# X1X1010/XequiNet

Hardware: AMD Instinct MI355X
Metric: edges/sec + achieved HBM GB/s, energy+force inference, QM9-shape batch (higher is better)
Workload: dtype f32

## Files before the change

### include/xeq.h

```cpp
#ifndef XEQ_H
#define XEQ_H
#include <stdint.h>

#ifdef __cplusplus
extern "C" {
#endif

enum { XEQ_F32 = 0, XEQ_F64 = 1 };
enum { XEQ_RBF_BESSEL = 0, XEQ_RBF_GAUSSIAN = 1, XEQ_RBF_EXPBERN = 2, XEQ_RBF_EXPNORM = 3 };
enum { XEQ_CUTOFF_COSINE = 0, XEQ_CUTOFF_POLYNOMIAL = 1 };
enum {
  XEQ_OK = 0,
  XEQ_ERR_INVALID_ARGUMENT = 1,
  XEQ_ERR_LAUNCH = 2,
  XEQ_ERR_UNSUPPORTED = 3
};

int xeq_version(void);
const char* xeq_last_error(void);
int64_t xeq_launch_count(void);
int64_t xeq_launch_names(int64_t first, char* buf, int64_t cap);


int xeq_csr_rowptr(const int64_t* keys, int64_t n_keys, int64_t n_rows, int32_t* rowptr, void* stream);
// ... 119 lines not shown
int xeq_wgrad_chunks(int64_t n, int m, int k);
int xeq_wgrad(const void* a, int64_t lda, const void* b, int64_t ldb, int64_t n, int m, int k, int with_bias, int n_chunks, void* parts,
              void* stream);

int xeq_load_padded_batch(int dtype, const void* pos, const int32_t* z, const int64_t* ptr, const int64_t* batch, int64_t n,
                          int64_t g, int64_t n_cap, int64_t g_cap, double pad0, double spacing, void* pos_out, int32_t* z_out,
                          int64_t* ptr_out, int64_t* batch_out, void* stream);
int xeq_load_padded_batch_z64(int dtype, const void* pos, const int64_t* z, const int64_t* ptr, const int64_t* batch, int64_t n, int64_t g,
                              int64_t n_cap, int64_t g_cap, double pad0, double spacing, void* pos_out, int32_t* z_out,
                              int64_t* ptr_out, int64_t* batch_out, void* stream);
int xeq_load_padded_shard(int dtype, const void* pos, const void* z, int z_is_int64, const int64_t* ptr, const int64_t* batch, int64_t n,
                          int64_t g, int64_t atom_offset, int64_t graph_offset, int64_t n_cap, int64_t g_cap, double pad0, double spacing,
                          void* pos_out, int32_t* z_out, int64_t* ptr_out, int64_t* batch_out, void* stream);

#define XEQ_COPY_MANY_MAX 16
int xeq_copy_many(int n, const void* const* src, void* const* dst, const int64_t* bytes, void* stream);
int xeq_compare_many(int n, const void* const* a, const void* const* b, const int64_t* bytes, int32_t gen, int32_t* flag, void* stream);

int xeq_tensor_product(int dtype, const void* x1, const void* x2, int64_t n, int dim1, int dim2, int dim_out, int n_paths,
                       const int32_t* paths, const void* cg, const int32_t* cg_off, int cg_floats, const void* weight, int64_t weight_stride,
                       const int32_t* w_off, const double* coeff, void* out, void* stream);
int64_t xeq_tensor_product_wgrad_chunks(int64_t n);
int xeq_tensor_product_wgrad(int dtype, const void* x1, const void* x2, const void* g, int64_t n, int dim1, int dim2, int dim_out, int n_paths,
                             const int32_t* paths, const void* cg, const int32_t* cg_off, const int32_t* w_off, const int32_t* w_numel, int w_total,
                             const double* coeff, int shared, void* parts, void* stream);

int xeq_tensor_product_path(int dtype, const void* x1, const void* x2, int64_t n, int dim1, int dim2, int dim_out, int off1,
                            int off2, int off_out, int mul1, int mul2, int mul_out, int l1, int l2, int l3, int mode,
                            const void* cg, const void* weight, int64_t weight_stride, double coeff, void* out, void* stream);


int xeq_message_fwd(int dtype, int64_t n_nodes, int64_t n_edges, const int32_t* rowptr, const int32_t* perm,
                    const int64_t* nbr, const void* vec, const void* h, const void* xhat, const void* s_in,
                    const void* x_in, const void* w_rbf, const void* b_rbf, const void* p0, const void* p1,
                    int rbf_kind, int cutoff_kind, int num_basis, double cutoff, int node_dim,
                    const int32_t mul[3], void* s_out, void* x_out, int xhat_layout, void* stream);

int xeq_message_bwd(int dtype, int64_t n_nodes, int64_t n_edges, const int32_t* n_rowptr, const int32_t* n_perm,
                    const int64_t* center, const void* vec, const void* h, const void* xhat, const void* grad_s,
                    const void* grad_x, const void* w_rbf, const void* b_rbf, const void* p0, const void* p1,
                    int rbf_kind, int cutoff_kind, int num_basis, double cutoff, int node_dim,
                    const int32_t mul[3], void* grad_h, void* grad_xhat, void* grad_vec, int xhat_layout,
                    void* stream);

int xeq_message_param_grad_parts(int64_t n_nodes);
int xeq_message_param_grad(int dtype, int64_t n_nodes, int64_t n_edges, const int32_t* n_rowptr, const int32_t* n_perm,
                           const int64_t* center, const void* vec, const void* h, const void* xhat, const void* grad_s,
                           const void* grad_x, const void* p0, const void* p1, int rbf_kind, int cutoff_kind, int num_basis,
                           double cutoff, int node_dim, const int32_t mul[3], int xhat_layout, int n_parts, void* parts,
                           void* stream);

int xeq_message_param_grad_mc_supported(int dtype, int rbf_kind, int num_basis, int node_dim, const int32_t mul[3]);
int xeq_param_basis_width(int rbf_kind, int num_basis);
int xeq_message_param_grad_mc_parts(int64_t n_edges, int node_dim, const int32_t mul[3]);
int xeq_param_basis(const void* vec, int64_t n_edges, int rbf_kind, int cutoff_kind, int num_basis, double cutoff, const void* p0,
                    const void* p1, void* tab, void* stream);
int xeq_message_param_grad_mc(int64_t n_nodes, int64_t n_edges, const int64_t* center, const int64_t* nbr, const void* tab, const void* h,
                              const void* xhat, const void* grad_s, const void* grad_x, int rbf_kind, int num_basis, int node_dim,
                              const int32_t mul[3], int xhat_layout, int grad_x_layout, const int32_t* n_valid, int n_parts, void* parts,
                              void* stream);
int xeq_norm_param_grad_chunks(int64_t n_nodes);
int xeq_norm_param_grad(const void* s, const void* x, const void* stats, const void* g_shat, int64_t ld_gs, const void* g_xhat_bt,
                        int64_t n_nodes, int node_dim, const int32_t mul[3], int n_chunks, void* parts, void* stream);
int xeq_to_bt(const void* x, int64_t n_nodes, const int32_t mul[3], void* out, void* stream);

int xeq_train_norm(int dtype, int reverse, int64_t n, const void* s, const void* s_tan, const void* x, const void* x_tan, const void* ln_w,
                   const void* ln_b, const void* eq_w, const void* eq_b, const void* g_s, const void* g_x, int node_dim,
                   const int32_t mul[3], double eps_ln, double eps_eq, int xhat_layout, void* out_s, void* out_x, void* rows, void* stream);
int xeq_train_uv(int dtype, int reverse, int64_t n, const void* const uv[3], const void* const uv_tan[3], const void* g, const int32_t mul[3],
                 double eps, void* out, void* const d_uv[3], void* stream);
int xeq_train_out(int dtype, int reverse, int64_t n, const void* const uv[3], const void* const uv_tan[3], const void* a, const void* a_tan,
                  const void* inner, const void* inner_tan, const void* g_s, const void* g_x, int node_dim, const int32_t mul[3],
                  void* out0, void* out1, void* const d_uv[3], void* stream);

int xeq_train_edge_supported(int dtype, int rbf_kind, int cutoff_kind, int num_basis);
int xeq_train_edge(int dtype, int reverse, int64_t n_edges, const void* vec, const void* vec_tan, const void* g_rec, const void* g_rec_tan,
                   int rbf_kind, int cutoff_kind, int num_basis, double cutoff, const void* p0, const void* p1, void* out, void* stream);

#define XEQ_FAMILY_WQ 0
#define XEQ_FAMILY_SB 1
#define XEQ_FAMILY_GENERIC 3
int xeq_message_auto_family(int dtype, int64_t n_nodes, int64_t n_edges, int num_basis, int node_dim, const int32_t mul[3]);
int xeq_message_wq_edges_per_stream(int64_t n_nodes, int64_t n_edges);

int xeq_edge_basis_width(int num_basis);
int xeq_message_sb_fits(int64_t n_nodes, int64_t n_edges, int num_basis, int node_dim, const int32_t mul[3]);
int xeq_edge_basis(int dtype, const void* vec, int64_t n_edges, int rbf_kind, int cutoff_kind, int num_basis,
                   double cutoff, const void* p0, const void* p1, void* basis, void* dbasis, void* stream);
int xeq_message_fwd_sb(int dtype, int64_t n_nodes, int64_t n_edges, const int32_t* rowptr, const int32_t* perm,
                       const int64_t* nbr, const void* basis, const void* h, const void* xhat, const void* s_in,
                       const void* x_in, const void* w_rbf, const void* b_rbf, int num_basis, int node_dim,
                       const int32_t mul[3], void* s_out, void* x_out, int xhat_layout, void* stream);
int xeq_message_bwd_sb(int dtype, int64_t n_nodes, int64_t n_edges, const int32_t* n_rowptr, const int32_t* n_perm,
                       const int64_t* center, const void* basis, const void* dbasis, const void* h, const void* xhat,
                       const void* grad_s, const void* grad_x, const void* w_rbf, const void* b_rbf, int num_basis,
                       int node_dim, const int32_t mul[3], void* grad_h, void* grad_xhat, void* grad_vec,
                       int xhat_layout, void* stream);

#define XEQ_SB_Y0_ZERO 8
#define XEQ_SB_ACCUM_VEC 16
#define XEQ_SB_Q_ACCUMULATE 16
#define XEQ_SB_NO_GY 32
int xeq_message_bwd_sbq(int dtype, int64_t n_nodes, int64_t n_edges, const int32_t* n_rowptr, const int32_t* n_perm,
                        const int64_t* center, const void* basis, const void* h, const void* xhat, const void* grad_s,
                        const void* grad_x, const void* w_rbf, const void* b_rbf, int num_basis, int node_dim,
                        const int32_t mul[3], void* grad_h, void* grad_xhat, void* q, void* gy, int flags, void* stream);
int xeq_message_fwd_sb_pair(int dtype, int64_t n_nodes, int64_t n_edges, const int32_t* rowptr, const int32_t* perm, const int64_t* nbr,
                            const void* basis, const void* basis_u, const void* h, const void* u_h, const void* xhat, const void* u_xhat,
                            const void* s_in, const void* x_in, const void* w_rbf, const void* b_rbf, int num_basis, int node_dim,
                            const int32_t mul[3], void* s_out, void* x_out, int xhat_layout, void* stream);
int xeq_message_bwd_sbq_pair(int dtype, int64_t n_nodes, int64_t n_edges, const int32_t* n_rowptr, const int32_t* n_perm,
                             const int64_t* center, const void* basis, const void* basis_u, const void* h, const void* u_h, const void* xhat,
                             const void* u_xhat, const void* grad_s, const void* grad_x, const void* w_rbf, const void* b_rbf, int num_basis,
                             int node_dim, const int32_t mul[3], void* grad_h, void* grad_xhat, void* q, void* gy, int flags, void* stream);
int xeq_zero_rows_from(void* buf, int64_t row_words, int64_t n_rows, const int32_t* n_valid, void* stream);
int xeq_message_q_wgrad_chunks(int64_t n_edges);
int xeq_message_q_wgrad(int dtype, const void* q, const void* basis, int64_t n_edges, int num_basis, int node_dim, const int32_t mul[3],
                        int n_chunks, void* parts, void* stream);

int xeq_message_wq_supported(int num_basis, int node_dim, const int32_t mul[3]);
int xeq_message_wq_fits(int64_t n_nodes, int64_t n_edges, int num_basis, int node_dim, const int32_t mul[3]);
int64_t xeq_message_wq_pcap(int64_t n_nodes, int64_t n_edges);
int xeq_message_wq_waves(void);
int xeq_message_wq_record_floats_for(int num_basis);
int xeq_message_wq_record_floats(void);
int64_t xeq_message_wq_plan_workspace(int64_t n_nodes);
int64_t xeq_message_wq_win_ints(int n_ranges);
int xeq_message_wq_plan(const int32_t* rowptr, const int32_t* perm, const int64_t* owner, const int64_t* gather,
                        int64_t n_nodes, int64_t n_edges, int n_ranges, void* workspace, int64_t workspace_bytes,
                        int32_t* qptr, int32_t* pgath, int32_t* peid, int32_t* qinfo, int32_t* sq, int32_t* sn, int32_t* win,
                        void* stream);
int xeq_edge_basis_wq(const void* vec, int64_t n_nodes, int64_t n_edges, const int32_t* qptr, const int32_t* peid,
                      int rbf_kind, int cutoff_kind, int num_basis, double cutoff, const void* p0, const void* p1,
                      void* basis, void* dbasis, void* stream);
int xeq_message_fwd_wq(int64_t n_nodes, int64_t n_edges, int n_ranges, const int32_t* sq, const int32_t* sn, const int32_t* win,
                       const int32_t* c_rowptr, const int32_t* pgath, const int32_t* qinfo, const void* basis, const void* h,
                       const void* xhat, const void* s_in, const void* x_in, const void* w_rbf, const void* b_rbf,
                       int num_basis, int node_dim, const int32_t mul[3], void* s_out, void* x_out, int xhat_layout,
                       void* stream);
int64_t xeq_message_wq_parts_floats(int64_t n_nodes, int64_t n_edges, const int32_t mul[3]);
#define XEQ_XHAT_HIGHER_L_ZERO 2
#define XEQ_WQ_MIRROR_WALK 4
#define XEQ_WQ_PACKED_WEIGHTS 64
int64_t xeq_message_wq_packed_weight_floats(int num_basis, int node_dim, const int32_t mul[3]);
int xeq_message_wq_pack_weights(const void* w_rbf, const void* b_rbf, int num_basis, int node_dim, const int32_t mul[3], void* packed,
                                void* stream);
int xeq_message_bwd_wq(int64_t n_nodes, int64_t n_edges, int n_ranges, const int32_t* sq, const int32_t* sn, const int32_t* win,
                       const int32_t* n_rowptr, const int32_t* pgath, const int32_t* qinfo, const void* basis,
                       const void* dbasis, const void* h, const void* xhat, const void* grad_s, const void* grad_x,
                       const void* w_rbf, const void* b_rbf, int num_basis, int node_dim, const int32_t mul[3], void* grad_h,
                       void* grad_xhat, void* parts, int xhat_layout, void* stream);
int xeq_message_wq_table_max_rows(void);
int xeq_message_wq_first_table(int family, int64_t table_rows, int training, int per_node_front);
int xeq_edge_basis_wq_table(const void* vec, int64_t n_nodes, int64_t n_edges, const int32_t* qptr, const int32_t* peid,
                            int rbf_kind, int cutoff_kind, int num_basis, double cutoff, const void* p0, const void* p1,
                            void* basis, void* dbasis, const int32_t* pgath, const int32_t* qinfo, const void* z, int z_is_int64,
                            int64_t table_rows, int32_t* slot_rows, int32_t* quad_rows, void* stream);
int xeq_message_fwd_wq_table(int64_t n_nodes, int64_t n_edges, int n_ranges, const int32_t* sq, const int32_t* sn, const int32_t* win,
                             const int32_t* c_rowptr, const int32_t* slot_rows, const int32_t* qinfo, const void* basis,
                             const void* h_table, const void* xhat0_table, int64_t table_rows, const void* s_in, const void* x_in,
                             const void* w_rbf, const void* b_rbf, int num_basis, int node_dim, const int32_t mul[3], void* s_out,
                             void* x_out, int xhat_layout, void* stream);
int xeq_message_bwd_wq_table(int64_t n_nodes, int64_t n_edges, int n_ranges, const int32_t* sq, const int32_t* sn, const int32_t* win,
                             const int32_t* n_rowptr, const int32_t* pgath, const int32_t* qinfo, const int32_t* quad_rows,
                             const void* basis, const void* dbasis, const void* h_table, const void* xhat0_table, int64_t table_rows,
                             const void* grad_s, const void* grad_x, const void* w_rbf, const void* b_rbf, int num_basis, int node_dim,
// ... 257 lines not shown
```

### xequinet_amd/csrc/xeq_message_wq.hip

```cpp
#include "xeq_message_wq.h"

#include <hipcub/hipcub.hpp>

namespace xeq {

struct QuadCount {
  const int32_t* rowptr;
  int64_t n;
  __host__ __device__ int32_t operator()(int64_t i) const {
    if (i >= n) return 0;
    const int32_t deg = rowptr[i + 1] - rowptr[i];
    return deg > 0 ? (deg + 3) >> 2 : 1;
  }
};
__global__ void __launch_bounds__(SCAN_WG_THREADS) k_wq_quad_scan(const QuadCount op, int32_t* __restrict__ qptr) {
  extern __shared__ int32_t scan_lds[];
  const int32_t total = wg_scan_lds(op, op.n, scan_lds);
#pragma unroll 4
  for (int64_t i = threadIdx.x; i < op.n; i += SCAN_WG_THREADS) qptr[i] = scan_lds[i];
  if (threadIdx.x == 0) qptr[op.n] = total;
}

__global__ void k_wq_fill(int64_t E, int64_t n_nodes, const int32_t* __restrict__ rowptr, const int32_t* __restrict__ perm,
                          const int64_t* __restrict__ owner, const int64_t* __restrict__ gather,
                          const int32_t* __restrict__ qptr, int32_t* __restrict__ pgath, int32_t* __restrict__ peid,
                          uint32_t* __restrict__ qinfo) {
  const int64_t s = (int64_t)blockIdx.x * blockDim.x + threadIdx.x;
  if (s >= E) {
    const int64_t n = s - E;
    if (n < n_nodes && rowptr[n] == rowptr[n + 1]) {
      const int64_t q0 = qptr[n];
      for (int i = 0; i < 4; ++i) {
        pgath[4 * q0 + i] = (int32_t)n;
        peid[4 * q0 + i] = -1;
      }
      qinfo[q0] = (uint32_t)n | WQ_FIRST | WQ_LAST;
    }
    return;
  }
  if (s >= rowptr[n_nodes]) return;
  const int32_t eid = perm ? perm[s] : (int32_t)s;
  const int64_t n = owner[eid];
  const int32_t r0 = rowptr[n], deg = rowptr[n + 1] - r0, k = (int32_t)(s - r0), q0 = qptr[n], nq = (deg + 3) >> 2;
  const int64_t p = 4 * (int64_t)q0 + k;
  pgath[p] = (int32_t)gather[eid];
  peid[p] = eid;
  if (k == deg - 1)
    for (int64_t pp = p + 1; pp < 4 * (int64_t)(q0 + nq); ++pp) {
      pgath[pp] = (int32_t)n;
      peid[pp] = -1;
    }
  if ((k & 3) == 0) {
    const int32_t g = k >> 2;
    qinfo[q0 + g] = (uint32_t)n | (g == 0 ? WQ_FIRST : 0u) | (g == nq - 1 ? WQ_LAST : 0u);
  }
}

__global__ void k_wq_streams(const int32_t* __restrict__ qptr, int64_t N, int n_ranges, int32_t* __restrict__ sq,
                             int32_t* __restrict__ sn) {
  const int k = blockIdx.x * blockDim.x + threadIdx.x;
  if (k > 2 * n_ranges) return;
  const int64_t Q = qptr[N];
  if (k == 2 * n_ranges) {
    sq[k] = (int32_t)Q;
    sn[k] = (int32_t)N;
    return;
  }
  const int64_t target = (int64_t)k * Q / (2 * n_ranges);
  int64_t lo = 0, hi = N;
  while (lo < hi) {
    const int64_t mid = (lo + hi) >> 1;
    if (qptr[mid] >= target) hi = mid;
    else lo = mid + 1;
  }
  sq[k] = qptr[lo];
  sn[k] = (int32_t)lo;
}

__global__ void k_wq_windows(const int32_t* __restrict__ sq, const int32_t* __restrict__ pgath, int n_ranges, int n_steps, int mult,
                             int32_t* __restrict__ win) {
  const int step = blockIdx.x, lane = threadIdx.x;
  if (step >= n_steps) return;
  const int k0 = min(2 * WQ_WAVES * mult * step, 2 * n_ranges), k1 = min(k0 + 2 * WQ_WAVES * mult, 2 * n_ranges);
  const int64_t p0 = 4 * (int64_t)sq[k0], p1 = 4 * (int64_t)sq[k1];
  int lo = 0x7fffffff, hi = -1;
  for (int64_t p = p0 + lane; p < p1; p += 64) {
    const int g = pgath[p];
    lo = g < lo ? g : lo;
    hi = g > hi ? g : hi;
  }
#pragma unroll
  for (int o = 32; o > 0; o >>= 1) {
    const int l2 = __shfl_xor(lo, o, 64), h2 = __shfl_xor(hi, o, 64);
    lo = l2 < lo ? l2 : lo;
    hi = h2 > hi ? h2 : hi;
  }
  if (lane == 0) {
    win[2 * step] = hi >= 0 ? lo : 0;
    win[2 * step + 1] = hi >= 0 ? hi - lo + 1 : 0;
  }
}

__device__ __forceinline__ void wq_record_piece(const float* __restrict__ vec, const int32_t* __restrict__ peid, int64_t p, int grp,
                                                const RadialSpec& rs, const float* __restrict__ p0, const float* __restrict__ p1,
                                                float* __restrict__ out, float* __restrict__ dout, int tailw, bool bftail) {
  const int yoff = WQ_TAIL + 2 * tailw;
  const int32_t e = peid[p];
  const f32x4 zero = {0.f, 0.f, 0.f, 0.f};
  if (e < 0) {
    if (grp < 2) {
#pragma unroll
      for (int c = 0; c < 3; ++c) {
        *reinterpret_cast<f32x4*>(out + 12 * grp + 4 * c) = zero;
        if (dout) *reinterpret_cast<f32x4*>(dout + 12 * grp + 4 * c) = zero;
      }
    } else if (grp < 4) {
      for (int c = 0; c < tailw; c += 4) {
        *reinterpret_cast<f32x4*>(out + WQ_TAIL + tailw * (grp - 2) + c) = zero;
        if (dout) *reinterpret_cast<f32x4*>(dout + WQ_TAIL + tailw * (grp - 2) + c) = zero;
      }
    } else {
      *reinterpret_cast<f32x4*>(out + yoff + 4 * (grp - 4)) = zero;
      if (dout) *reinterpret_cast<f32x4*>(dout + yoff + 4 * (grp - 4)) = zero;
    }
    return;
  }
  const float rc = (float)rs.cutoff;
  const EdgeGeom<float> g = edge_geom<float>(vec[3 * (int64_t)e], vec[3 * (int64_t)e + 1], vec[3 * (int64_t)e + 2]);
  const int B = rs.num_basis;
  if (grp >= 4) {
    float y1[3], y2[5];
    sph_harm_l12<float>(g, y1, y2);
    const f32x4 v = grp == 4 ? f32x4{y1[0], y1[1], y1[2], y2[0]} : f32x4{y2[1], y2[2], y2[3], y2[4]};
    *reinterpret_cast<f32x4*>(out + yoff + 4 * (grp - 4)) = v;
    if (dout) *reinterpret_cast<f32x4*>(dout + yoff + 4 * (grp - 4)) = v;
    return;
  }
  float f, df;
// ... 421 lines not shown
  }
  __syncthreads();
  int* tbl = tbl_all[threadIdx.x >> 6];
#ifdef XEQ_WQ_ROLE_TIME_FWD
  unsigned long long rr0_;
  asm volatile("s_memrealtime %0\n\ts_waitcnt lgkmcnt(0)" : "=s"(rr0_)::"memory");
#endif
  if (un.l == 0) wq_fwd_role<1, KS, false, !XZ, TAB>(a, s_beg, s_end, un, rec, h, xhat, s_in, x_in, wl, s_out, x_out, tbl, win);
  else if (un.l == 1) wq_fwd_role<3, KS, XZ, !XZ, TAB>(a, s_beg, s_end, un, rec, h, xhat, s_in, x_in, wl, s_out, x_out, tbl, win);
  else wq_fwd_role<5, KS, XZ, !XZ, TAB>(a, s_beg, s_end, un, rec, h, xhat, s_in, x_in, wl, s_out, x_out, tbl, win);
#ifdef XEQ_WQ_ROLE_TIME_FWD
  if (threadIdx.x == 0 && blockIdx.x < 8192) {
    unsigned long long rr1_;
    unsigned hw, xcc;
    asm volatile("s_waitcnt vmcnt(0)\n\ts_memrealtime %0\n\ts_getreg_b32 %1, hwreg(HW_REG_HW_ID)\n\ts_getreg_b32 %2, hwreg(HW_REG_XCC_ID)\n\ts_waitcnt lgkmcnt(0)"
                 : "=s"(rr1_), "=s"(hw), "=s"(xcc)::"memory");
    g_wq_wg[4 * blockIdx.x + 0] = hw | ((unsigned long long)un.l << 32);
    g_wq_wg[4 * blockIdx.x + 1] = xcc;
    g_wq_wg[4 * blockIdx.x + 2] = rr0_;
    g_wq_wg[4 * blockIdx.x + 3] = rr1_;
  }
#endif
}


}

using namespace xeq;

extern "C" {

int xeq_message_wq_table_max_rows(void) { return WQ_TAB_MAX_ROWS; }

int xeq_message_wq_supported(int num_basis, int node_dim, const int32_t mul[3]) { return wq_supported(num_basis, node_dim, mul) ? 1 : 0; }

int xeq_message_wq_fits(int64_t n_nodes, int64_t n_edges, int num_basis, int node_dim, const int32_t mul[3]) {
  return wq_supported(num_basis, node_dim, mul) && n_nodes < (1ll << 30) && wq_fits(n_nodes, n_edges, node_dim, mul) ? 1 : 0;
}

int64_t xeq_message_wq_pcap(int64_t n_nodes, int64_t n_edges) { return wq_pcap(n_nodes, n_edges); }

int xeq_message_wq_waves(void) { return WQ_WAVES; }

int xeq_message_wq_record_floats(void) { return wq_recf(4); }
int xeq_message_wq_record_floats_for(int num_basis) { return wq_recf(wq_ks(num_basis)); }

int64_t xeq_message_wq_plan_workspace(int64_t n_nodes) {
  size_t temp = 0;
  QuadCount op{nullptr, n_nodes};
  hipcub::CountingInputIterator<int64_t> cnt(0);
  hipcub::TransformInputIterator<int32_t, QuadCount, hipcub::CountingInputIterator<int64_t>> it(cnt, op);
  if (hipcub::DeviceScan::ExclusiveSum(nullptr, temp, it, (int32_t*)nullptr, (int)(n_nodes + 1)) != hipSuccess) return -1;
  return (int64_t)temp + 256;
}

int xeq_message_wq_plan(const int32_t* rowptr, const int32_t* perm, const int64_t* owner, const int64_t* gather,
                        int64_t n_nodes, int64_t n_edges, int n_ranges, void* workspace, int64_t workspace_bytes,
                        int32_t* qptr, int32_t* pgath, int32_t* peid, int32_t* qinfo, int32_t* sq, int32_t* sn, int32_t* win,
                        void* stream) {
  XEQ_CHECK_ARG(n_nodes >= 0 && n_edges >= 0 && n_ranges >= 1 && n_nodes < (1ll << 30) && n_edges < (1ll << 31), "xeq_message_wq_plan: bad sizes");
  const int64_t need = xeq_message_wq_plan_workspace(n_nodes);
  XEQ_CHECK_ARG(need >= 0 && workspace_bytes >= need, "xeq_message_wq_plan: workspace of %lld bytes, need %lld", (long long)workspace_bytes, (long long)need);
  QuadCount op{rowptr, n_nodes};
  if (n_nodes <= SCAN_WG_MAX_ITEMS) {
    static const bool attr_ok = hipFuncSetAttribute((const void*)k_wq_quad_scan, hipFuncAttributeMaxDynamicSharedMemorySize,
                                                    (int)wg_scan_lds_bytes(SCAN_WG_MAX_ITEMS)) == hipSuccess;
    XEQ_CHECK_ARG(attr_ok, "xeq_message_wq_plan: cannot reserve LDS for the quad scan");
    hipLaunchKernelGGL(k_wq_quad_scan, dim3(1), dim3(SCAN_WG_THREADS), wg_scan_lds_bytes(n_nodes), (hipStream_t)stream, op, qptr);
    XEQ_CHECK_LAUNCH("xeq_message_wq_plan (quad scan)");
  } else {
    hipcub::CountingInputIterator<int64_t> cnt(0);
    hipcub::TransformInputIterator<int32_t, QuadCount, hipcub::CountingInputIterator<int64_t>> it(cnt, op);
    size_t temp = (size_t)workspace_bytes;
    if (hipcub::DeviceScan::ExclusiveSum(workspace, temp, it, qptr, (int)(n_nodes + 1), (hipStream_t)stream) != hipSuccess) {
      xeq::set_error("xeq_message_wq_plan: scan failed");
      return XEQ_ERR_LAUNCH;
    }
  }
  if (n_edges + n_nodes > 0) {
    hipLaunchKernelGGL(k_wq_fill, dim3((unsigned)((n_edges + n_nodes + 255) / 256)), dim3(256), 0, (hipStream_t)stream, n_edges, n_nodes,
                       rowptr, perm, owner, gather, (const int32_t*)qptr, pgath, peid, (uint32_t*)qinfo);
    XEQ_CHECK_LAUNCH("xeq_message_wq_plan (fill)");
  }
  const int n = 2 * n_ranges + 1;
  hipLaunchKernelGGL(k_wq_streams, dim3((unsigned)((n + 255) / 256)), dim3(256), 0, (hipStream_t)stream, (const int32_t*)qptr,
                     n_nodes, n_ranges, sq, sn);
  XEQ_CHECK_LAUNCH("xeq_message_wq_plan (streams)");
  const int n_steps = wq_class_steps(n_ranges, 1);
  hipLaunchKernelGGL(k_wq_windows, dim3((unsigned)n_steps), dim3(64), 0, (hipStream_t)stream, (const int32_t*)sq,
                     (const int32_t*)pgath, n_ranges, n_steps, 1, win);
  XEQ_CHECK_LAUNCH("xeq_message_wq_plan (windows)");
  const int mlong = wq_long_mult(n_edges, n_ranges);
  if (mlong > 1) {
    const int n_long = wq_class_steps(n_ranges, mlong);
    hipLaunchKernelGGL(k_wq_windows, dim3((unsigned)n_long), dim3(64), 0, (hipStream_t)stream, (const int32_t*)sq,
                       (const int32_t*)pgath, n_ranges, n_long, mlong, win + 2 * n_steps);
    XEQ_CHECK_LAUNCH("xeq_message_wq_plan (windows, long class)");
  }
  return XEQ_OK;
}

int64_t xeq_message_wq_win_ints(int n_ranges) {
  return 2 * ((int64_t)wq_class_steps(n_ranges, 1) + (int64_t)wq_class_steps(n_ranges, 2) + 1);
}

static int wq_edge_basis(const void* vec, int64_t n_nodes, int64_t n_edges, const int32_t* qptr, const int32_t* peid,
                         int rbf_kind, int cutoff_kind, int num_basis, double cutoff, const void* p0, const void* p1,
                         void* basis, void* dbasis, const WqTableIndex& ti, void* stream) {
  XEQ_CHECK_ARG(n_edges >= 0 && n_nodes >= 0 && num_basis >= 1 && num_basis <= 31 && cutoff > 0, "xeq_edge_basis_wq: bad sizes");
  XEQ_CHECK_ARG(rbf_kind >= XEQ_RBF_BESSEL && rbf_kind <= XEQ_RBF_EXPNORM, "xeq_edge_basis_wq: rbf kernel %d is not implemented", rbf_kind);
  XEQ_CHECK_ARG(rbf_kind == XEQ_RBF_BESSEL || p1 != nullptr, "xeq_edge_basis_wq: this radial basis needs its second parameter array (std / logc / mu)");
  XEQ_CHECK_ARG(cutoff_kind == XEQ_CUTOFF_COSINE || cutoff_kind == XEQ_CUTOFF_POLYNOMIAL, "xeq_edge_basis_wq: cutoff function %d is not implemented", cutoff_kind);
  if (n_edges == 0 && n_nodes == 0) return XEQ_OK;
  const int64_t pcap = wq_pcap(n_nodes, n_edges), total = (pcap + WQ_REC_SLOTS - 1) / WQ_REC_SLOTS * 256;
  const int ks = wq_ks(num_basis);
  XEQ_CHECK_ARG(pcap * wq_recf(ks) < (1ll << 31) * 2, "xeq_edge_basis_wq: too many edges for 32-bit record offsets (shard the batch)");
  RadialSpec rs{rbf_kind, cutoff_kind, num_basis, cutoff};
  hipLaunchKernelGGL(k_wq_records, dim3((unsigned)((total + 255) / 256)), dim3(256), 0, (hipStream_t)stream, (const float*)vec,
                     peid, qptr, n_nodes, pcap, rs, (const float*)p0, (const float*)p1, (float*)basis, (float*)dbasis, wq_recf(ks), wq_tailw(ks), wq_bftail(ks) ? 1 : 0, ti);
  XEQ_CHECK_LAUNCH("xeq_edge_basis_wq");
  return XEQ_OK;
}
int xeq_edge_basis_wq(const void* vec, int64_t n_nodes, int64_t n_edges, const int32_t* qptr, const int32_t* peid,
                      int rbf_kind, int cutoff_kind, int num_basis, double cutoff, const void* p0, const void* p1,
                      void* basis, void* dbasis, void* stream) {
  return wq_edge_basis(vec, n_nodes, n_edges, qptr, peid, rbf_kind, cutoff_kind, num_basis, cutoff, p0, p1, basis, dbasis, WqTableIndex{}, stream);
}
int xeq_edge_basis_wq_table(const void* vec, int64_t n_nodes, int64_t n_edges, const int32_t* qptr, const int32_t* peid,
                            int rbf_kind, int cutoff_kind, int num_basis, double cutoff, const void* p0, const void* p1,
                            void* basis, void* dbasis, const int32_t* pgath, const int32_t* qinfo, const void* z, int z_is_int64,
                            int64_t table_rows, int32_t* slot_rows, int32_t* quad_rows, void* stream) {
  XEQ_CHECK_ARG(pgath && qinfo && z && slot_rows && quad_rows && table_rows >= 1, "xeq_edge_basis_wq_table: NULL argument / empty table");
  const WqTableIndex ti{z, z_is_int64, table_rows, pgath, (const uint32_t*)qinfo, slot_rows, quad_rows};
  return wq_edge_basis(vec, n_nodes, n_edges, qptr, peid, rbf_kind, cutoff_kind, num_basis, cutoff, p0, p1, basis, dbasis, ti, stream);
}

static int wq_ks_template(int num_basis) {
  const int ks = wq_ks(num_basis);
  return ks <= 1 ? 1 : (ks <= 3 ? 3 : (ks <= 4 ? 4 : 8));
}
int64_t xeq_message_wq_packed_weight_floats(int num_basis, int node_dim, const int32_t mul[3]) {
  if (!wq_supported(num_basis, node_dim, mul)) return -1;
  const int kst = wq_ks_template(num_basis);
  const int64_t per_unit = 3 * (int64_t)(3 * 64 * 4 + (wq_bftail(kst) ? 3 * 64 * 4 : kst * 64));
  return per_unit * (mul[0] / 32 + mul[1] / 32 + mul[2] / 32);
}
int xeq_message_wq_pack_weights(const void* w_rbf, const void* b_rbf, int num_basis, int node_dim, const int32_t mul[3], void* packed,
                                void* stream) {
  WqArgs a{};
  int rcode = wq_check("xeq_message_wq_pack_weights", 0, 0, 1, num_basis, node_dim, mul, a);
  if (rcode != XEQ_OK) return rcode;
  XEQ_CHECK_ARG(w_rbf && b_rbf && packed, "xeq_message_wq_pack_weights: NULL argument");
  const int nunits = a.nu[0] + a.nu[1] + a.nu[2];
  const dim3 grid((unsigned)nunits);
  switch (wq_ks_template(num_basis)) {
    case 1: hipLaunchKernelGGL(k_wq_pack_weights<1>, grid, dim3(256), 0, (hipStream_t)stream, a, (const float*)w_rbf, (const float*)b_rbf, (float*)packed); break;
    case 3: hipLaunchKernelGGL(k_wq_pack_weights<3>, grid, dim3(256), 0, (hipStream_t)stream, a, (const float*)w_rbf, (const float*)b_rbf, (float*)packed); break;
    case 4: hipLaunchKernelGGL(k_wq_pack_weights<4>, grid, dim3(256), 0, (hipStream_t)stream, a, (const float*)w_rbf, (const float*)b_rbf, (float*)packed); break;
    default: hipLaunchKernelGGL(k_wq_pack_weights<8>, grid, dim3(256), 0, (hipStream_t)stream, a, (const float*)w_rbf, (const float*)b_rbf, (float*)packed); break;
  }
  XEQ_CHECK_LAUNCH("xeq_message_wq_pack_weights");
  return XEQ_OK;
}

static int wq_message_fwd(int64_t n_nodes, int64_t n_edges, int n_ranges, const int32_t* sq, const int32_t* sn, const int32_t* win,
                          const int32_t* c_rowptr, const int32_t* pgath, const int32_t* qinfo, const void* basis, const void* h,
                          const void* xhat, const void* s_in, const void* x_in, const void* w_rbf, const void* b_rbf,
                          int num_basis, int node_dim, const int32_t mul[3], void* s_out, void* x_out, int xhat_layout,
                          const int32_t* slot_rows, int64_t table_rows, void* stream) {
  WqArgs a{};
  int rcode = wq_check("xeq_message_fwd_wq", n_nodes, n_edges, n_ranges, num_basis, node_dim, mul, a);
  if (rcode != XEQ_OK) return rcode;
  if (n_nodes == 0) return XEQ_OK;
  a.sq = sq;
  a.sn = sn;
  a.rowptr = c_rowptr;
  a.pgath = slot_rows ? slot_rows : pgath;
  a.tab_rows = (int)table_rows;
  a.qinfo = (const uint32_t*)qinfo;
  a.xl = xhat_layout & 1;
  a.packed_w = (xhat_layout & XEQ_WQ_PACKED_WEIGHTS) ? 1 : 0;
// ... 38 lines not shown
```

### xequinet_amd/lib.py

```python
from __future__ import annotations

import ctypes
import os
from ctypes import c_char_p, c_double, c_int, c_int32, c_int64, c_uint64, c_void_p
from typing import Optional

import torch

_HERE = os.path.dirname(os.path.abspath(__file__))
LIB_PATH = os.environ.get("XEQ_LIB_PATH") or os.path.join(_HERE, "libxeq_hip.so")

XEQ_F32, XEQ_F64 = 0, 1
COPY_MANY_MAX = 16
MD_CHUNK = 256
MD_NVE, MD_LANGEVIN, MD_BERENDSEN, MD_PURPOSE_LANGEVIN, MD_PURPOSE_MAXWELL = 0, 1, 2, 0, 1
NPT_BOX, NPT_CELL, NPT_INV, NPT_CELL_NEXT, NPT_INV_NEXT, NPT_MU, NPT_P, NPT_V = 40, 0, 9, 18, 27, 36, 37, 38
FIRE_FRESH, FIRE_ACTIVE, FIRE_CONVERGED = 0, 1, 2
VIB_MAX_DIM, VIB_MAX_SWEEPS = 96, 30
VIB_ROTORS = ("atom", "linear", "nonlinear")
SB_ACCUM_VEC = 16
XHAT_HIGHER_L_ZERO = 2
SB_Y0_ZERO = 8
SB_Q_ACCUMULATE = 16
SB_NO_GY = 32
# ... 42 lines not shown
    "xeq_launch_names": [c_int64, c_char_p, c_int64],
    "xeq_csr_rowptr": [_P, c_int64, c_int64, _P, _P],
    "xeq_csr_by_key_workspace": [c_int64, c_int64],
    "xeq_csr_by_key": [_P, c_int64, c_int64, _P, c_int64, _P, _P, _P],
    "xeq_csr_by_key_bounded": [_P, c_int64, c_int64, _P, _P, c_int64, _P, _P, _P],
    "xeq_exclusive_scan_i32": [_P, c_int64, _P, _P],
    "xeq_exclusive_scan_i32_workspace": [c_int64],
    "xeq_exclusive_scan_i32_ws": [_P, c_int64, _P, _P, c_int64, _P],
    "xeq_reverse_edge_map": [_P, c_int64, c_int64, _P, _P, _P],
    "xeq_reverse_edge_map_pbc": [c_int, _P, _P, c_int64, c_int64, _P, _P, _P],
    "xeq_radius_graph_count": [c_int, _P, _P, c_int64, c_int64, c_double, _P, _P],
    "xeq_radius_graph_fill": [c_int, _P, _P, c_int64, c_int64, c_double, _P, c_int64, _P, _P],
    "xeq_radius_graph_bin_ids": [c_int, _P, _P, c_int64, c_int64, _P, _P, _P, _P, _P, _P],
    "xeq_radius_graph_count_cl": [c_int, _P, _P, c_int64, c_int64, c_double, _P, _P, _P, _P, _P, _P, _P, _P],
    "xeq_radius_graph_fill_cl": [c_int, _P, _P, c_int64, c_int64, c_double, _P, _P, _P, _P, _P, _P, _P, c_int64, _P, _P, _P],
    "xeq_pbc_image_counts": [c_int, _P, c_int64, _I3, c_double, _I3],
    "xeq_pbc_tables_host": [c_int, _P, c_int64, _I3, c_double, _P, c_int64],
    "xeq_pbc_wrap": [c_int, _P, _P, c_int64, c_int64, _P, _P, _I3, _P, _P, _P],
    "xeq_radius_graph_pbc_count": [c_int, _P, _P, c_int64, c_int64, _P, c_int64, c_double, _P, _P],
    "xeq_radius_graph_pbc_fill": [c_int, _P, _P, c_int64, c_int64, _P, _P, _P, c_int64, c_double, _P, c_int64, _P, _P, _P],
    "xeq_radius_graph_pbc_count_pruned": [c_int, _P, _P, c_int64, c_int64, _P, c_int64, c_double, _P, _P, _I3, _P, _P],
    "xeq_radius_graph_pbc_fill_pruned": [c_int, _P, _P, c_int64, c_int64, _P, _P, _P, c_int64, c_double, _P, _P, _I3, _P, c_int64,
                                         _P, _P, _P],
    "xeq_radius_graph_pbc_bin_ids": [c_int, _P, _P, c_int64, c_int64, _P, _P, _P, _P, _P],
    "xeq_radius_graph_pbc_count_cl": [c_int, _P, _P, c_int64, c_int64, _P, c_int64, c_double, _P, _P, _I3, _P, _P, _P, _P, _P, _P],
    "xeq_radius_graph_pbc_fill_cl": [c_int, _P, _P, c_int64, c_int64, _P, _P, _P, c_int64, c_double, _P, _P, _I3, _P, _P, _P, _P,
                                     _P, c_int64, _P, _P, _P, _P],
    "xeq_edge_vectors_fwd": [c_int, _P, _P, c_int64, _P, _P, _P, _P, _P, _P],
    "xeq_edge_vectors_bwd": [c_int, _P, c_int64, _P, _P, _P, _P, _P, _P],
    "xeq_sph_harm_fwd": [c_int, _P, c_int64, _I3, c_int, _P, _P],
    "xeq_sph_harm_bwd": [c_int, _P, _P, c_int64, _I3, c_int, _P, _P],
    "xeq_radial_fwd": [c_int, _P, c_int64, c_int, c_int, c_int, c_double, _P, _P, _P, _P, _P],
    "xeq_elementwise_tp_fwd": [c_int, _P, _P, c_int64, c_int64, _I3, _P, _P],
    "xeq_channel_dot_fwd": [c_int, _P, _P, c_int64, _I3, _P, _P],
    "xeq_eqln_fwd": [c_int, _P, _P, _P, c_int64, _I3, c_double, _P, _P],
    "xeq_eqln_bwd": [c_int, _P, _P, _P, c_int64, _I3, c_double, _P, _P],
    "xeq_segment_sum": [c_int, _P, _P, c_int64, c_int64, _P, _P],
    "xeq_linear_supported": [c_int, c_int, c_int],
    "xeq_mfma_order_probe": [_P, _P, _P, _P],
    "xeq_linear_fwd": [_P, c_int64, c_int64, c_int, _P, _P, c_int, c_int, c_int, _P, _P, c_int64, _P],
    "xeq_head_dot": [_P, c_int64, c_int, _P, _P, _P, _P],
    "xeq_head_bwd_hidden": [_P, c_int64, c_int, _P, _P, _P, _P],
    "xeq_head_supported": [c_int, c_int, c_int],
    "xeq_head_fwd": [_P, c_int64, c_int64, c_int, c_int, _P, _P, _P, _P, _P, _P, _P],
    "xeq_head_bwd": [_P, c_int64, c_int, _P, c_int64, _P, c_int64, _P, _P, _P],
    "xeq_electronic_supported": [c_int, c_int],
    "xeq_electronic_fwd": [c_int, _P, c_int64, c_int64, c_int, _P, c_int64, _P, _P, _P, _P, _P, _P, _P, _P, _P],
    "xeq_first_block_front": [_P, c_int, c_int64, c_int64, _P, _P, _P, c_int, c_int, c_int64, _P, _P, _P, _P],
    "xeq_rowptr_from_degrees": [_P, c_int64, c_int64, _P, _P, _P, _P],
    "xeq_rowptr_from_degrees_max": [],
    "xeq_wgrad_chunks": [c_int64, c_int, c_int],
    "xeq_wgrad": [_P, c_int64, _P, c_int64, c_int64, c_int, c_int, c_int, c_int, _P, _P],
    "xeq_load_padded_batch": [c_int, _P, _P, _P, _P, c_int64, c_int64, c_int64, c_int64, c_double, c_double, _P, _P, _P, _P, _P],
    "xeq_load_padded_batch_z64": [c_int, _P, _P, _P, _P, c_int64, c_int64, c_int64, c_int64, c_double, c_double, _P, _P, _P, _P, _P],
    "xeq_load_padded_shard": [c_int, _P, _P, c_int, _P, _P, c_int64, c_int64, c_int64, c_int64, c_int64, c_int64, c_double, c_double, _P, _P, _P, _P, _P],
    "xeq_copy_many": [c_int, ctypes.POINTER(c_void_p), ctypes.POINTER(c_void_p), ctypes.POINTER(c_int64), _P],
    "xeq_compare_many": [c_int, ctypes.POINTER(c_void_p), ctypes.POINTER(c_void_p), ctypes.POINTER(c_int64), ctypes.c_int32, _P, _P],
    "xeq_tensor_product_path": [c_int, _P, _P, c_int64, c_int, c_int, c_int, c_int, c_int, c_int, c_int, c_int, c_int, c_int, c_int,
                                c_int, c_int, _P, _P, c_int64, c_double, _P, _P],
    "xeq_tensor_product": [c_int, _P, _P, c_int64, c_int, c_int, c_int, c_int, ctypes.POINTER(ctypes.c_int32), _P, ctypes.POINTER(ctypes.c_int32),
                           c_int, _P, c_int64, ctypes.POINTER(ctypes.c_int32), ctypes.POINTER(c_double), _P, _P],
    "xeq_tensor_product_wgrad": [c_int, _P, _P, _P, c_int64, c_int, c_int, c_int, c_int, ctypes.POINTER(ctypes.c_int32), _P,
                                 ctypes.POINTER(ctypes.c_int32), ctypes.POINTER(ctypes.c_int32), ctypes.POINTER(ctypes.c_int32), c_int,
                                 ctypes.POINTER(c_double), c_int, _P, _P],
    "xeq_tensor_product_wgrad_chunks": [c_int64],
    "xeq_scatter_add": [c_int, _P, _P, c_int64, c_int64, _P, c_int64, _P],
    "xeq_message_fwd": [c_int, c_int64, c_int64, _P, _P, _P, _P, _P, _P, _P, _P, _P, _P, _P, _P,
                        c_int, c_int, c_int, c_double, c_int, _I3, _P, _P, c_int, _P],
    "xeq_message_bwd": [c_int, c_int64, c_int64, _P, _P, _P, _P, _P, _P, _P, _P, _P, _P, _P, _P,
                        c_int, c_int, c_int, c_double, c_int, _I3, _P, _P, _P, c_int, _P],
    "xeq_message_param_grad_parts": [c_int64],
    "xeq_message_param_grad": [c_int, c_int64, c_int64, _P, _P, _P, _P, _P, _P, _P, _P, _P, _P, c_int, c_int, c_int, c_double, c_int,
                               _I3, c_int, c_int, _P, _P],
    "xeq_message_param_grad_mc_supported": [c_int, c_int, c_int, c_int, _I3],
    "xeq_param_basis_width": [c_int, c_int],
    "xeq_message_param_grad_mc_parts": [c_int64, c_int, _I3],
    "xeq_param_basis": [_P, c_int64, c_int, c_int, c_int, c_double, _P, _P, _P, _P],
    "xeq_message_param_grad_mc": [c_int64, c_int64, _P, _P, _P, _P, _P, _P, _P, c_int, c_int, c_int, _I3, c_int, c_int, _P, c_int, _P, _P],
    "xeq_to_bt": [_P, c_int64, _I3, _P, _P],
    "xeq_norm_param_grad_chunks": [c_int64],
    "xeq_norm_param_grad": [_P, _P, _P, _P, c_int64, _P, c_int64, c_int, _I3, c_int, _P, _P],
    "xeq_message_auto_family": [c_int, c_int64, c_int64, c_int, c_int, _I3],
    "xeq_message_wq_edges_per_stream": [c_int64, c_int64],
    "xeq_edge_basis_width": [c_int],
    "xeq_edge_basis": [c_int, _P, c_int64, c_int, c_int, c_int, c_double, _P, _P, _P, _P, _P],
    "xeq_message_fwd_sb": [c_int, c_int64, c_int64, _P, _P, _P, _P, _P, _P, _P, _P, _P, _P, c_int, c_int, _I3, _P, _P, c_int, _P],
    "xeq_message_bwd_sbq": [c_int, c_int64, c_int64, _P, _P, _P, _P, _P, _P, _P, _P, _P, _P, c_int, c_int, _I3, _P, _P, _P, _P, c_int, _P],
    "xeq_message_q_wgrad": [c_int, _P, _P, c_int64, c_int, c_int, _I3, c_int, _P, _P],
    "xeq_message_q_wgrad_chunks": [c_int64],
    "xeq_train_norm": [c_int, c_int, c_int64, _P, _P, _P, _P, _P, _P, _P, _P, _P, _P, c_int, _I3, c_double, c_double, c_int, _P, _P, _P, _P],
    "xeq_train_uv": [c_int, c_int, c_int64, _P, _P, _P, _I3, c_double, _P, _P, _P],
    "xeq_train_out": [c_int, c_int, c_int64, _P, _P, _P, _P, _P, _P, _P, _P, c_int, _I3, _P, _P, _P, _P],
    "xeq_train_edge_supported": [c_int, c_int, c_int, c_int],
    "xeq_train_edge": [c_int, c_int, c_int64, _P, _P, _P, _P, c_int, c_int, c_int, c_double, _P, _P, _P, _P],
    "xeq_zero_rows_from": [_P, c_int64, c_int64, _P, _P],
    "xeq_message_fwd_sb_pair": [c_int, c_int64, c_int64, _P, _P, _P, _P, _P, _P, _P, _P, _P, _P, _P, _P, _P, c_int, c_int, _I3, _P, _P, c_int, _P],
    "xeq_message_bwd_sbq_pair": [c_int, c_int64, c_int64, _P, _P, _P, _P, _P, _P, _P, _P, _P, _P, _P, _P, _P, c_int, c_int, _I3, _P, _P, _P, _P, c_int, _P],
    "xeq_message_bwd_sb": [c_int, c_int64, c_int64, _P, _P, _P, _P, _P, _P, _P, _P, _P, _P, _P, c_int, c_int, _I3, _P, _P, _P,
                           c_int, _P],
    "xeq_message_sb_fits": [c_int64, c_int64, c_int, c_int, _I3],
    "xeq_message_wq_supported": [c_int, c_int, _I3],
    "xeq_message_wq_fits": [c_int64, c_int64, c_int, c_int, _I3],
    "xeq_message_wq_pcap": [c_int64, c_int64],
    "xeq_message_wq_waves": [],
    "xeq_message_wq_record_floats": [],
    "xeq_message_wq_record_floats_for": [c_int],
    "xeq_message_wq_plan_workspace": [c_int64],
    "xeq_message_wq_win_ints": [c_int],
    "xeq_message_wq_plan": [_P, _P, _P, _P, c_int64, c_int64, c_int, _P, c_int64, _P, _P, _P, _P, _P, _P, _P, _P],
    "xeq_edge_basis_wq": [_P, c_int64, c_int64, _P, _P, c_int, c_int, c_int, c_double, _P, _P, _P, _P, _P],
    "xeq_message_fwd_wq": [c_int64, c_int64, c_int, _P, _P, _P, _P, _P, _P, _P, _P, _P, _P, _P, _P, _P, c_int, c_int, _I3,
                           _P, _P, c_int, _P],
    "xeq_message_wq_table_max_rows": [],
    "xeq_message_wq_first_table": [c_int, c_int64, c_int, c_int],
    "xeq_edge_basis_wq_table": [_P, c_int64, c_int64, _P, _P, c_int, c_int, c_int, c_double, _P, _P, _P, _P, _P, _P, _P, c_int, c_int64, _P, _P, _P],
    "xeq_message_fwd_wq_table": [c_int64, c_int64, c_int, _P, _P, _P, _P, _P, _P, _P, _P, _P, c_int64, _P, _P, _P, _P, c_int, c_int, _I3,
                                 _P, _P, c_int, _P],
    "xeq_message_bwd_wq_table": [c_int64, c_int64, c_int, _P, _P, _P, _P, _P, _P, _P, _P, _P, _P, _P, c_int64, _P, _P, _P, _P, c_int, c_int,
                                 _I3, _P, c_int, _P],
    "xeq_message_wq_parts_floats": [c_int64, c_int64, _I3],
    "xeq_message_bwd_wq": [c_int64, c_int64, c_int, _P, _P, _P, _P, _P, _P, _P, _P, _P, _P, _P, _P, _P, _P, c_int, c_int,
                           _I3, _P, _P, _P, c_int, _P],
    "xeq_message_wq_packed_weight_floats": [c_int, c_int, _I3],
    "xeq_message_wq_pack_weights": [_P, _P, c_int, c_int, _I3, _P, _P],
    "xeq_message_wq_edge_grad": [_P, c_int64, c_int64, _P, _P, _P, _I3, _P, _P, _P],
    "xeq_message_wq_edge_grad_sum": [_P, c_int64, c_int64, _P, _P, _P, _I3, c_int, ctypes.POINTER(c_void_p), _P, _P],
    "xeq_norm_fwd": [c_int, _P, _P, _P, _P, _P, _P, c_int64, c_int, _I3, c_int, _P, c_int64, _P, _P, _P],
    "xeq_norm_bwd": [c_int, _P, _P, _P, _P, _P, c_int64, c_int, _I3, c_int, _P, c_int64, _P, _P, _P, _P, _P, _P],
    "xeq_uv_reduce_fwd": [c_int, _P, c_int64, _I3, c_double, _P, c_int64, c_int, _P, _P],
    "xeq_uv_reduce_bwd": [c_int, _P, _P, _P, c_int64, c_int, c_int64, _I3, c_double, _P, _P, _P, _P],
    "xeq_update_out_fwd": [c_int, _P, _P, _P, _P, _P, c_int64, c_int, _I3, _P, _P, _P],
    "xeq_update_out_bwd": [c_int, _P, _P, _P, _P, _P, c_int64, c_int, _I3, _P, _P, _P, _P],
    "xeq_update_uv_supported": [c_int, c_int, _I3],
    "xeq_update_uv_fwd": [_P, _P, _P, _P, _P, _P, c_int64, c_int, _I3, c_int, _P, _P, _P, c_int, c_double, _P, c_int64, _P, _P, _P, _P],
    "xeq_update_uv_bwd": [_P, _P, _P, c_int64, _P, _P, _P, c_int64, _P, _P, _P, _P, _P, c_int64, c_int, _I3, c_int, _P, _P, _P, c_double,
                          _P, _P, _P, _P],
    "xeq_mlp2_supported": [c_int, c_int, c_int, c_int],
    "xeq_node_tile_split": [c_int64, c_int, ctypes.POINTER(c_int64)],
    "xeq_mlp_packed_floats": [c_int, c_int],
    "xeq_mlp_pack": [_P, _P, c_int, c_int, c_int, _P, _P],
    "xeq_mlp2_fwd": [_P, c_int64, c_int64, c_int, _P, _P, c_int, _P, _P, c_int64, _P],
    "xeq_mlp2_bwd": [_P, c_int64, c_int64, c_int, _P, _P, _P, c_int, _P, c_int64, _P],
    "xeq_mlp2h_supported": [c_int, c_int, c_int, c_int],
    "xeq_mlp2h_fwd": [c_int, _P, c_int64, c_int64, c_int, c_int, _P, _P, c_int, _P, _P, c_int64, _P],
    "xeq_mlp2h_bwd": [c_int, _P, c_int64, c_int64, c_int, c_int, _P, _P, _P, c_int, _P, c_int64, _P],
    "xeq_mlp2_and_linear": [c_int, _P, c_int64, c_int64, c_int, _P, _P, c_int, _P, _P, c_int64, _P, c_int64, c_int, _P, c_int, _P, c_int64, _P],
    "xeq_pack_epoch": [],
    "xeq_pack_epoch_bump": [],
    "xeq_rowptr_guard": [_P, c_int64, c_int64, _P, _P, _P],
    "xeq_node_block_supported": [c_int, c_int, _I3],
    "xeq_node_block_fwd_tiles": [c_int],
    "xeq_node_block_rows": [c_int64],
    "xeq_node_block_auto": [c_int64],
    "xeq_small_rows_limit": [],
    "xeq_node_block_set_waves": [c_int],
    "xeq_node_block_pack_fwd": [_P, _P, _P, _P, _P, _P, _P, _P, _P, _P],
    "xeq_node_block_fwd": [c_int64, _P, _P, _P, _P, _P, _P, _P, _P, _P, c_double, _P, _P, _P, _P, _P, _P, _P, _P, _P, _P, _P, _P, _P, _P, _P,
                           _P, _P, _P, _P, _P],
    "xeq_node_block_linear_test": [_P, c_int64, _P, c_int, c_int, _P, _P, _P],
    "xeq_node_block_bwd_tiles": [c_int, c_int],
    "xeq_node_block_pack_bwd": [_P, _P, _P, _P, _P, _P, _P, _P, c_int, _P, _P],
    "xeq_node_block_bwd": [c_int64, _P, _P, _P, _P, _P, _P, _P, _P, _P, _P, _P, _P, _P, _P, _P, _P, _P, _P, _P, c_double, _P, _P, _P, _P, _P,
                           _P, _P, _P],
    "xeq_painn_supported": [c_int, c_int, c_int],
    "xeq_painn_few_rows_limit": [],
    "xeq_painn_filter_packed_floats": [c_int],
# ... 150 lines not shown
```

Baseline: 181.8 million.

## Cut WQ streams by per-stream tile capacity instead of equal quad counts

Replaces the equal-quad-count stream partition with a per-block minimax cut. Each workgroup loads its slice of the quad prefix sums into LDS, computes greedy next-cut pointers and pointer-doubling hops, then searches for the smallest per-stream tile cap that covers its node range. The aim is to balance work across streams in whole quad tiles and avoid streams that overrun. In exchange the planning kernel gets heavier, with iterative search and many barriers. A host reference path and an env override to fall back to the old cut are also added.

Result: no change. 184.0 million, median of 3 (+1.2%).

```diff
diff --git a/include/xeq.h b/include/xeq.h
--- a/include/xeq.h
+++ b/include/xeq.h
@@ -225,6 +225,8 @@
 #define XEQ_FAMILY_GENERIC 3
 int xeq_message_auto_family(int dtype, int64_t n_nodes, int64_t n_edges, int num_basis, int node_dim, const int32_t mul[3]);
 int xeq_message_wq_edges_per_stream(int64_t n_nodes, int64_t n_edges);
+int xeq_message_wq_stream_tiles(void);
+int xeq_message_wq_stream_cut(const int32_t* qptr, int64_t n_nodes, int n_ranges, int tiles, int32_t* sq, int32_t* sn);
 
 int xeq_edge_basis_width(int num_basis);
 int xeq_message_sb_fits(int64_t n_nodes, int64_t n_edges, int num_basis, int node_dim, const int32_t mul[3]);
diff --git a/xequinet_amd/csrc/xeq_message_wq.hip b/xequinet_amd/csrc/xeq_message_wq.hip
--- a/xequinet_amd/csrc/xeq_message_wq.hip
+++ b/xequinet_amd/csrc/xeq_message_wq.hip
@@ -1,6 +1,9 @@
 #include "xeq_message_wq.h"
 
 #include <hipcub/hipcub.hpp>
+
+#include <cstring>
+#include <vector>
 
 namespace xeq {
 
@@ -54,6 +57,157 @@
     const int32_t g = k >> 2;
     qinfo[q0 + g] = (uint32_t)n | (g == 0 ? WQ_FIRST : 0u) | (g == nq - 1 ? WQ_LAST : 0u);
   }
+}
+
+__host__ __device__ __forceinline__ int64_t wq_cut_lower_bound(const int32_t* __restrict__ qptr, int64_t N, int64_t target) {
+  int64_t lo = 0, hi = N;
+  while (lo < hi) {
+    const int64_t mid = (lo + hi) >> 1;
+    if (qptr[mid] >= target) hi = mid;
+    else lo = mid + 1;
+  }
+  return lo;
+}
+
+constexpr int WQ_CUT_TILES = 6;
+constexpr int WQ_CUT_BLOCK_SLOTS = 2 * WQ_WAVES * 16;
+constexpr int WQ_CUT_MAX_NODES = 2048;
+constexpr int WQ_CUT_THREADS = 256;
+struct WqCutScratch {
+  int32_t* lq;
+  int32_t* nxt;
+  int32_t* hop2;
+  int32_t* hop4;
+  int32_t* pos;
+  int32_t* sh;
+};
+#if defined(__HIP_DEVICE_COMPILE__)
+#define XEQ_WQ_CUT_SYNC() __syncthreads()
+__device__ __forceinline__ void wq_cut_bounds_wg(const int32_t* __restrict__ qptr, int64_t N, int64_t t0, int64_t t1, int32_t* sh,
+                                                 int64_t& n0, int64_t& n1) {
+  const int tid = (int)threadIdx.x, half = tid >> 7, r = tid & 127;
+  const int64_t target = half ? t1 : t0;
+  int64_t lo = 0, hi = N;
+  for (int64_t bound = N; bound > 0; bound = (bound + 127) / 128 - 1) {
+    const int64_t span = hi - lo, step = (span + 127) / 128, p = lo + r * step;
+    const bool below = span > 0 && p < hi && qptr[p] < target;
+    const unsigned long long m = __ballot(below);
+    if ((tid & 63) == 0) sh[tid >> 6] = __popcll(m);
+    __syncthreads();
+    const int f = sh[2 * half] + sh[2 * half + 1];
+    __syncthreads();
+    if (span > 0) {
+      if (f == 0) {
+        hi = lo;
+      } else {
+        const int64_t nhi = lo + f * step;
+        lo = lo + (f - 1) * step + 1;
+        hi = nhi < hi ? nhi : hi;
+      }
+    }
+  }
+  if (r == 0) sh[half] = (int32_t)lo;
+  __syncthreads();
+  n0 = sh[0];
+  n1 = sh[1];
+  __syncthreads();
+}
+#else
+#define XEQ_WQ_CUT_SYNC() ((void)0)
+#endif
+__host__ __device__ inline void wq_cut_block(const int32_t* __restrict__ qptr, int64_t N, int n_ranges, int tiles, int block, int tid,
+                                             int nthr, const WqCutScratch& sc, int32_t* __restrict__ sq, int32_t* __restrict__ sn) {
+  const int64_t S = 2 * (int64_t)n_ranges, Q = qptr[N];
+  const int64_t k0 = (int64_t)block * WQ_CUT_BLOCK_SLOTS, k1 = k0 + WQ_CUT_BLOCK_SLOTS < S ? k0 + WQ_CUT_BLOCK_SLOTS : S;
+  const int ns = (int)(k1 - k0);
+  if (k1 == S && tid == 0) {
+    sq[S] = (int32_t)Q;
+    sn[S] = (int32_t)N;
+  }
+  int64_t n0, n1;
+#if defined(__HIP_DEVICE_COMPILE__)
+  wq_cut_bounds_wg(qptr, N, k0 * Q / S, k1 * Q / S, sc.sh, n0, n1);
+#else
+  n0 = wq_cut_lower_bound(qptr, N, k0 * Q / S);
+  n1 = wq_cut_lower_bound(qptr, N, k1 * Q / S);
+#endif
+  const int nb = (int)(n1 - n0 > WQ_CUT_MAX_NODES ? WQ_CUT_MAX_NODES + 1 : n1 - n0);
+  if (tiles < 1 || nb > WQ_CUT_MAX_NODES) {
+    for (int64_t k = k0 + tid; k < k1; k += nthr) {
+      const int64_t n = wq_cut_lower_bound(qptr, N, k * Q / S);
+      sq[k] = qptr[n];
+      sn[k] = (int32_t)n;
+    }
+    return;
+  }
+  for (int i = tid; i <= nb; i += nthr) sc.lq[i] = qptr[n0 + i];
+  XEQ_WQ_CUT_SYNC();
+  auto cut_at = [&](int64_t t) {
+    const int64_t cap = 4 * t;
+    for (int i = tid; i < nb; i += nthr) {
+      const int64_t limit = (int64_t)sc.lq[i] + cap;
+      int a = i + 1, b = (int)(cap < nb - i ? i + cap : nb);
+      if (sc.lq[a] <= limit)
+        while (a < b) {
+          const int mid = (a + b + 1) >> 1;
+          if (sc.lq[mid] <= limit) a = mid;
+          else b = mid - 1;
+        }
+      sc.nxt[i] = a;
+    }
+    if (tid == 0) sc.nxt[nb] = nb;
+    XEQ_WQ_CUT_SYNC();
+    for (int i = tid; i <= nb; i += nthr) sc.hop2[i] = sc.nxt[sc.nxt[i]];
+    XEQ_WQ_CUT_SYNC();
+    for (int i = tid; i <= nb; i += nthr) sc.hop4[i] = sc.hop2[sc.hop2[i]];
+    XEQ_WQ_CUT_SYNC();
+    if (tid == 0)
+      for (int j = 0, p = 0; j < ns; j += 4, p = sc.hop4[p]) sc.pos[j] = p;
+    XEQ_WQ_CUT_SYNC();
+    for (int j = 4 * tid; j < ns; j += 4 * nthr)
+      for (int u = 1, p = sc.pos[j]; u < 4 && j + u < ns; ++u) sc.pos[j + u] = p = sc.nxt[p];
+    XEQ_WQ_CUT_SYNC();
+    const bool fits = sc.nxt[sc.pos[ns - 1]] == nb;
+    XEQ_WQ_CUT_SYNC();
+    return fits;
+  };
+  const int64_t mean_tiles = (Q + 4 * S - 1) / (4 * S);
+  const int64_t first = mean_tiles < 1 ? 1 : (mean_tiles < tiles ? mean_tiles : tiles);
+  if (!cut_at(first)) {
+    int64_t fail = first, step = 1, last;
+    for (;;) {
+      last = fail + step;
+      if (cut_at(last)) break;
+      fail = last;
+      step *= 2;
+    }
+    int64_t fit = last;
+    while (fit - fail > 1) {
+      last = (fit + fail) >> 1;
+      if (cut_at(last)) fit = last;
+      else fail = last;
+    }
+    if (last != fit) cut_at(fit);
+  }
+  for (int j = tid; j < ns; j += nthr) {
+    const int p = sc.pos[j];
+    sq[k0 + j] = sc.lq[p];
+    sn[k0 + j] = (int32_t)(n0 + p);
+  }
+}
+__global__ void __launch_bounds__(WQ_CUT_THREADS) k_wq_stream_cut(const int32_t* __restrict__ qptr, int64_t N, int n_ranges, int tiles,
+                                                       int32_t* __restrict__ sq, int32_t* __restrict__ sn) {
+  __shared__ int32_t lq[WQ_CUT_MAX_NODES + 1], nxt[WQ_CUT_MAX_NODES + 1], hop2[WQ_CUT_MAX_NODES + 1], hop4[WQ_CUT_MAX_NODES + 1],
+      pos[WQ_CUT_BLOCK_SLOTS], sh[4];
+  const WqCutScratch sc{lq, nxt, hop2, hop4, pos, sh};
+  wq_cut_block(qptr, N, n_ranges, tiles, (int)blockIdx.x, (int)threadIdx.x, (int)blockDim.x, sc, sq, sn);
+}
+static int wq_stream_tiles() {
+  const char* cut = getenv("XEQ_WQ_STREAM_CUT");
+  if (cut && strcmp(cut, "quads") == 0) return 0;
+  const char* env = getenv("XEQ_WQ_STREAM_TILES");
+  if (env && atoi(env) >= 1 && atoi(env) <= 64) return atoi(env);
+  return WQ_CUT_TILES;
 }
 
 __global__ void k_wq_streams(const int32_t* __restrict__ qptr, int64_t N, int n_ranges, int32_t* __restrict__ sq,
@@ -641,9 +795,13 @@
                        rowptr, perm, owner, gather, (const int32_t*)qptr, pgath, peid, (uint32_t*)qinfo);
     XEQ_CHECK_LAUNCH("xeq_message_wq_plan (fill)");
   }
-  const int n = 2 * n_ranges + 1;
-  hipLaunchKernelGGL(k_wq_streams, dim3((unsigned)((n + 255) / 256)), dim3(256), 0, (hipStream_t)stream, (const int32_t*)qptr,
-                     n_nodes, n_ranges, sq, sn);
+  const int n = 2 * n_ranges + 1, tiles = wq_stream_tiles();
+  if (tiles < 1)
+    hipLaunchKernelGGL(k_wq_streams, dim3((unsigned)((n + 255) / 256)), dim3(256), 0, (hipStream_t)stream, (const int32_t*)qptr,
+                       n_nodes, n_ranges, sq, sn);
+  else
+    hipLaunchKernelGGL(k_wq_stream_cut, dim3((unsigned)((2 * (int64_t)n_ranges + WQ_CUT_BLOCK_SLOTS - 1) / WQ_CUT_BLOCK_SLOTS)),
+                       dim3(WQ_CUT_THREADS), 0, (hipStream_t)stream, (const int32_t*)qptr, n_nodes, n_ranges, tiles, sq, sn);
   XEQ_CHECK_LAUNCH("xeq_message_wq_plan (streams)");
   const int n_steps = wq_class_steps(n_ranges, 1);
   hipLaunchKernelGGL(k_wq_windows, dim3((unsigned)n_steps), dim3(64), 0, (hipStream_t)stream, (const int32_t*)sq,
@@ -656,6 +814,19 @@
                        (const int32_t*)pgath, n_ranges, n_long, mlong, win + 2 * n_steps);
     XEQ_CHECK_LAUNCH("xeq_message_wq_plan (windows, long class)");
   }
+  return XEQ_OK;
+}
+
+int xeq_message_wq_stream_tiles(void) { return wq_stream_tiles(); }
+
+int xeq_message_wq_stream_cut(const int32_t* qptr, int64_t n_nodes, int n_ranges, int tiles, int32_t* sq, int32_t* sn) {
+  XEQ_CHECK_ARG(qptr != nullptr && sq != nullptr && sn != nullptr && n_nodes >= 0 && n_nodes < (1ll << 30) && n_ranges >= 1,
+                "xeq_message_wq_stream_cut: bad arguments");
+  std::vector<int32_t> lq(WQ_CUT_MAX_NODES + 1), nxt(WQ_CUT_MAX_NODES + 1), hop2(WQ_CUT_MAX_NODES + 1), hop4(WQ_CUT_MAX_NODES + 1),
+      pos(WQ_CUT_BLOCK_SLOTS), sh(4);
+  const WqCutScratch sc{lq.data(), nxt.data(), hop2.data(), hop4.data(), pos.data(), sh.data()};
+  const int64_t blocks = (2 * (int64_t)n_ranges + WQ_CUT_BLOCK_SLOTS - 1) / WQ_CUT_BLOCK_SLOTS;
+  for (int64_t b = 0; b < blocks; ++b) wq_cut_block(qptr, n_nodes, n_ranges, tiles, (int)b, 0, 1, sc, sq, sn);
   return XEQ_OK;
 }
 
diff --git a/xequinet_amd/lib.py b/xequinet_amd/lib.py
--- a/xequinet_amd/lib.py
+++ b/xequinet_amd/lib.py
@@ -148,6 +148,8 @@
     "xeq_norm_param_grad": [_P, _P, _P, _P, c_int64, _P, c_int64, c_int, _I3, c_int, _P, _P],
     "xeq_message_auto_family": [c_int, c_int64, c_int64, c_int, c_int, _I3],
     "xeq_message_wq_edges_per_stream": [c_int64, c_int64],
+    "xeq_message_wq_stream_tiles": [],
+    "xeq_message_wq_stream_cut": [_P, c_int64, c_int, c_int, _P, _P],
     "xeq_edge_basis_width": [c_int],
     "xeq_edge_basis": [c_int, _P, c_int64, c_int, c_int, c_int, c_double, _P, _P, _P, _P, _P],
     "xeq_message_fwd_sb": [c_int, c_int64, c_int64, _P, _P, _P, _P, _P, _P, _P, _P, _P, _P, c_int, c_int, _I3, _P, _P, c_int, _P],
```
